# peterbudai/redux

Measured on NVIDIA B200. Metric: encode+decode round-trip throughput of raw input (bit-exact), higher is better.
Workload: dtype u32

## Files before the change

### redux_b200/csrc/redux_capi.cu

```cuda
#include <cuda_runtime.h>

#include <algorithm>
#include <chrono>
#include <atomic>
#include <condition_variable>
#include <deque>
#include <mutex>
#include <cstdio>
#include <cstdlib>
#include <cstring>
#include <string>
#include <thread>
#include <vector>

#include "../../include/redux_b200.h"
#include "redux_batch_kernels.cuh"
#include "redux_common.cuh"
#include "redux_lane_codec.cuh"
#include "redux_lane_al.cuh"
#include "redux_generic_codec.cuh"
#include "redux_warp_codec.cuh"
#include "redux_split_encoder.cuh"
#include "redux_train.cuh"

// ... 142 lines not shown
        release();
        cudaError_t e = cudaHostAlloc((void **)&buf, piece_bytes * (size_t)slots, cudaHostAllocDefault);
        if (e != cudaSuccess) { buf = nullptr; return e; }
        piece = piece_bytes; n = slots;
        ev.assign((size_t)slots, nullptr); recorded.assign((size_t)slots, 0);
        for (auto &x : ev) if ((e = cudaEventCreateWithFlags(&x, cudaEventDisableTiming)) != cudaSuccess) return e;
        return cudaSuccess;
    }
    void release() {
        for (auto x : ev) if (x) cudaEventDestroy(x);
        ev.clear(); recorded.clear();
        if (buf) cudaFreeHost(buf);
        buf = nullptr; piece = 0; n = 0;
    }
    uint8_t *slot(int i) const { return buf + (size_t)i * piece; }
};

struct StagingConfig {
    int enable = 1;
    size_t min_bytes = (size_t)8 << 20;
    size_t piece_bytes = (size_t)8 << 20;
    int slots = 4;
    int threads = 0;
};

struct DeviceState {
    int device = 0;
    cudaStream_t stream = nullptr;
    cudaStream_t pipe[kPipeStreams] = {};
    cudaStream_t copy = nullptr;
    cudaStream_t h2d = nullptr;
    HostBuf pin_off, pin_status, pin_aux0, pin_aux1;
    DevBuf slots, sizes, flag;
    DevBuf st_in, st_off, st_bmod, st_out, st_ooff, st_status, st_aux0, st_aux1, st_roff;
    DevBuf split_hist, split_pairs;
    DevBuf gen_tabs, gen_init, gen_freq, gen_start, gen_magic;
    DevBuf train_rows, train_sample;
    uint8_t *text_lut = nullptr;
    DevBuf corpus; uint64_t corpus_len = 0;
    std::vector<MagicEntry> magics;
    bool smem_set = false;
    cudaEvent_t ws_busy = nullptr;
    bool ws_recorded = false;
    StageRing *ring_up = nullptr, *ring_down = nullptr;
};

}

struct TimedSpan { cudaEvent_t a, b; int kind; int device; };

struct ModelArgs { bool on = false; const uint32_t *freqs = nullptr; uint32_t n = 0; const uint32_t *block_model = nullptr; };

struct redux_ctx {
    std::vector<DeviceState> devs;
    int sched = REDUX_SCHED_AUTO;
    std::string last_error;
    uint64_t launches = 0;
    bool timing = false;
    ModelArgs models;
    std::vector<TimedSpan> spans;
    StagingConfig staging;
    CopyPool *pool = nullptr;
    std::atomic<uint64_t> kernels_launched{0};
    void note_kernel(int id) { kernels_launched.fetch_or((uint64_t)1 << id, std::memory_order_relaxed); }
};

// ... 233 lines not shown
{
    job.magic = magic; job.f = pl.f; job.c = pl.c;
    job.tcap = pl.pretrained ? (uint32_t)(((uint64_t)1 << pl.f) - 1 - kNsym) : pl.tcap;
    job.one = pl.c <= 32 ? 1u << (32 - pl.c) : 0u;
    job.init_tree = nullptr; job.count0 = kNsym; job.eof_freq = 1;
    job.models = pl.models;
    job.models.block_model = pl.models.start ? block_model : nullptr;
    job.gf_m = pl.gf_m; job.gf_sh = pl.gf_sh;
}

KernelId pick_encoder(const Plan &pl)
{
    const bool c32 = pl.c == 32;
    if (pl.warp) return pl.cls == kNarrow ? kEncWarpNarrow : pl.cls == kWide ? kEncWarpWide : kEncWarpHuge;
    if (!pl.aligned) return pl.wide_table ? kEncHugeU32 : kEncHugeU16;
    if (pl.lane_cls == kNarrow) return kEncNarrow;
    if (pl.lane_cls == kWide) return c32 ? kEncWideU32C32 : kEncWideU32;
    if (pl.wide_table) return c32 ? kEncWideDU32C32 : kEncWideDU32;
    if (pl.full_table) return c32 ? kEncWideDU16FullC32 : kEncWideDU16Full;
    return c32 ? kEncWideDU16C32 : kEncWideDU16;
}
KernelId pick_decoder(const Plan &pl)
{
    const bool c32 = pl.c == 32;
    if (pl.warp) return pl.cls == kNarrow ? kDecWarpNarrow : pl.cls == kHuge ? kDecWarpHuge : c32 ? kDecWarpWideC32 : kDecWarpWide;
    if (!pl.aligned) return pl.wide_table ? kDecHugeU32 : kDecHugeU16;
    if (pl.lane_cls == kNarrow) return pl.c <= 16 ? kDecNarrowStg : kDecNarrow;
    if (pl.lane_cls == kWide) return c32 ? kDecWideU32C32 : kDecWideU32;
    if (pl.wide_table) return c32 ? kDecWideDU32C32 : kDecWideDU32;
    if (pl.full_table) return c32 ? kDecWideDU16FullC32 : kDecWideDU16Full;
    return c32 ? kDecWideDU16C32 : kDecWideDU16;
}

#define RDX_LAUNCH_LANE(id, name, kernel, TW) case id: kernel<<<lane_grid, kLaneThreads, lane_smem<TW>(), s>>>(job); return true;
#define RDX_LAUNCH_WARP(id, name, kernel) case id: kernel<<<warp_grid, kWarpCtaThreads, 0, s>>>(job); return true;
bool launch_coder(KernelId id, const LaneEncJob &job, cudaStream_t s)
{
    const uint32_t lane_grid = (uint32_t)((job.n_blocks + kLaneThreads - 1) / kLaneThreads);
    const uint32_t warp_grid = (uint32_t)((job.n_blocks + kWarpCtaWarps - 1) / kWarpCtaWarps);
    switch (id) {
    RDX_LANE_ENCODERS(RDX_LAUNCH_LANE)
    RDX_WARP_ENCODERS(RDX_LAUNCH_WARP)
    default: return false;
    }
}
bool launch_coder(KernelId id, const LaneDecJob &job, cudaStream_t s)
{
    const uint32_t lane_grid = (uint32_t)((job.n_blocks + kLaneThreads - 1) / kLaneThreads);
    const uint32_t warp_grid = (uint32_t)((job.n_blocks + kWarpCtaWarps - 1) / kWarpCtaWarps);
    switch (id) {
    RDX_LANE_DECODERS(RDX_LAUNCH_LANE)
    RDX_WARP_DECODERS(RDX_LAUNCH_WARP)
    default: return false;
    }
}
#undef RDX_LAUNCH_LANE
#undef RDX_LAUNCH_WARP

int launch_encode_split(redux_ctx *ctx, DeviceState *d, const Plan &pl, const LaneEncJob &job, cudaStream_t s, KernelId *kid)
{
    if (!d) return fail(ctx, REDUX_INVALID_INPUT, "device is not part of this context");
    SplitJob sj;
    sj.in = job.in; sj.in_off = job.in_off; sj.n_blocks = job.n_blocks;
    sj.chunks_per_stream = (uint32_t)((pl.max_len + kSplitChunk - 1) / kSplitChunk);
    sj.pair_stride = (pl.max_len + 31) & ~(uint64_t)31;
    sj.tcap = pl.tcap;
    const uint64_t chunks = job.n_blocks * sj.chunks_per_stream;
    CU_TRY(ctx, d->split_hist.reserve(chunks * 256 * sizeof(uint32_t)));
    CU_TRY(ctx, d->split_pairs.reserve(job.n_blocks * sj.pair_stride * sizeof(uint2)));
    sj.hist = (uint32_t *)d->split_hist.p; sj.pairs = (uint2 *)d->split_pairs.p;
    split_hist_kernel<<<(uint32_t)chunks, 256, 0, s>>>(sj);
    split_scan_kernel<<<(uint32_t)job.n_blocks, 256, 0, s>>>(sj);
    split_model_kernel<<<(uint32_t)((chunks + kSplitModelWarps - 1) / kSplitModelWarps), kSplitModelWarps * 32, 0, s>>>(sj);
    const uint32_t grid = (uint32_t)job.n_blocks;
    if (pl.cls == kNarrow)   { split_coder_kernel<kNarrow, false><<<grid, 32, 0, s>>>(job, sj); *kid = kSplitNarrow; }
    else if (pl.c == 32)     { split_coder_kernel<kWide, true><<<grid, 32, 0, s>>>(job, sj);    *kid = kSplitWideC32; }
    else                     { split_coder_kernel<kWide, false><<<grid, 32, 0, s>>>(job, sj);   *kid = kSplitWide; }
    ctx->launches += 3;
    return REDUX_OK;
}

int check_kind(redux_ctx *ctx, int kind)
{
    if (kind != REDUX_MODEL_LINEAR && kind != REDUX_MODEL_TREE)
        return fail(ctx, REDUX_INVALID_INPUT, "unknown model kind");
    return REDUX_OK;
}

struct DeviceGuard {
// ... 91 lines not shown

extern "C" uint32_t redux_debug_div_by_range(uint64_t x, uint64_t range) { return div_by_range64(x, range); }

extern "C" uint64_t redux_debug_magic_divide(uint64_t n, uint64_t magic, uint32_t shift, int wide)
{
    if (wide == 2) { Magic64 g{magic, shift, 0}; return div_magic65(n, g); }
    if (wide == 3) { union { double f; uint64_t u; } cv; cv.u = magic; MagicD g; g.r = cv.f; return div_magicd(n, g); }
    if (wide) { Magic64 g{magic, shift, 0}; return div_magic64(n, g); }
    Magic32 g{(uint32_t)magic, shift};
    return div_magic32((uint32_t)n, g);
}

extern "C" void redux_debug_renorm(uint64_t low, uint64_t high, uint32_t c, uint32_t *n1, uint32_t *k,
                                   uint64_t *nl, uint64_t *nh)
{
    if (c <= 32) { Renorm<uint32_t> r = renorm<uint32_t>((uint32_t)low, (uint32_t)high, c); *n1 = r.n1; *k = r.k; *nl = r.low; *nh = r.high; }
    else         { Renorm<uint64_t> r = renorm<uint64_t>(low, high, c); *n1 = r.n1; *k = r.k; *nl = r.low; *nh = r.high; }
}

extern "C" void redux_debug_shard(uint64_t n_blocks, uint32_t n_devices, uint32_t g, uint64_t *first, uint64_t *count)
{
    const uint64_t a = n_blocks * g / n_devices, b = n_blocks * (g + 1) / n_devices;
    *first = a; *count = b - a;
}

extern "C" int redux_debug_lane_occupancy(int *enc_ctas_per_sm, int *dec_ctas_per_sm)
{
    if (!enc_ctas_per_sm || !dec_ctas_per_sm) return REDUX_INVALID_INPUT;
    if (configure_kernels() != cudaSuccess) { (void)cudaGetLastError(); return REDUX_CUDA_ERROR; }
    const size_t s16 = (size_t)kLaneWarpsPerCta * kTabNodes * 32 * 2 + kTabPadBytes;
    if (cudaOccupancyMaxActiveBlocksPerMultiprocessor(enc_ctas_per_sm, encode_lane_al_kernel<uint16_t, kNarrow, true, false>,
                                                      kLaneThreads, s16) != cudaSuccess ||
        cudaOccupancyMaxActiveBlocksPerMultiprocessor(dec_ctas_per_sm, decode_lane_al_kernel<uint16_t, kNarrow, true, false, true>,
                                                      kLaneThreads, s16) != cudaSuccess) {
        (void)cudaGetLastError();
        return REDUX_CUDA_ERROR;
    }
    return REDUX_OK;
}

extern "C" const char *redux_debug_kernel_name(int id)
{
#define RDX_KERNEL_NAME(id, name, ...) name,
    static const char *const names[] = { RDX_ALL_KERNELS(RDX_KERNEL_NAME) };
#undef RDX_KERNEL_NAME
    return id >= 0 && id < kKernelIdCount ? names[id] : nullptr;
}

extern "C" int redux_debug_launched_kernels(redux_ctx_t *ctx, uint64_t *mask, int reset)
{
    if (!ctx || !mask) return REDUX_INVALID_INPUT;
    *mask = reset ? ctx->kernels_launched.exchange(0) : ctx->kernels_launched.load();
    return REDUX_OK;
}

extern "C" void redux_generate_blocks_host(uint8_t *out, uint64_t first_block, uint64_t n_blocks,
                                           uint64_t block_len, uint64_t seed)
{
    redux_generate_blocks_host_ex(out, first_block, n_blocks, block_len, seed, nullptr, 0);
}

extern "C" void redux_generate_blocks_host_ex(uint8_t *out, uint64_t first_block, uint64_t n_blocks,
                                              uint64_t block_len, uint64_t seed, const uint8_t *corpus, uint64_t corpus_len)
{
    uint8_t lut[256];
    for (uint32_t u = 0; u < 256; ++u) lut[u] = text_symbol(u);
    const uint64_t groups = (block_len + 7) >> 3;
// ... 62 lines not shown
                          cudaStreamCreateWithFlags(&d.copy, cudaStreamNonBlocking) == cudaSuccess &&
                          cudaStreamCreateWithFlags(&d.h2d, cudaStreamNonBlocking) == cudaSuccess;
        for (int i = 0; i < kPipeStreams && streams_ok; ++i)
            streams_ok = cudaStreamCreateWithFlags(&d.pipe[i], cudaStreamNonBlocking) == cudaSuccess;
        if (!streams_ok || cudaStreamCreateWithFlags(&d.stream, cudaStreamNonBlocking) != cudaSuccess ||
            configure_kernels() != cudaSuccess ||
            cudaMalloc((void **)&d.text_lut, 256) != cudaSuccess ||
            cudaMemcpy(d.text_lut, lut, 256, cudaMemcpyHostToDevice) != cudaSuccess) {
            (void)cudaGetLastError();
            ctx->devs.push_back(d);
            redux_ctx_destroy(ctx);
            return REDUX_CUDA_ERROR;
        }
        ctx->devs.push_back(d);
    }
    *out = ctx;
    return REDUX_OK;
}

extern "C" void redux_ctx_destroy(redux_ctx_t *ctx)
{
    if (!ctx) return;
    for (auto &d : ctx->devs) {
        DeviceGuard g(d.device);
        cudaDeviceSynchronize();
        if (d.ws_busy) cudaEventDestroy(d.ws_busy);
        if (d.stream) cudaStreamDestroy(d.stream);
        if (d.copy) cudaStreamDestroy(d.copy);
        if (d.h2d) cudaStreamDestroy(d.h2d);
        for (int i = 0; i < kPipeStreams; ++i) if (d.pipe[i]) cudaStreamDestroy(d.pipe[i]);
        for (HostBuf *b : {&d.pin_off, &d.pin_status, &d.pin_aux0, &d.pin_aux1}) b->release();
        for (DevBuf *b : {&d.slots, &d.sizes, &d.flag, &d.st_in, &d.st_off, &d.st_bmod, &d.st_out, &d.st_ooff,
                          &d.st_status, &d.st_aux0, &d.st_aux1, &d.st_roff, &d.corpus, &d.gen_magic, &d.gen_tabs, &d.gen_init,
                          &d.gen_freq, &d.gen_start, &d.split_hist, &d.split_pairs, &d.train_rows, &d.train_sample}) b->release();
        for (auto &m : d.magics) cudaFree(m.ptr);
        if (d.text_lut) cudaFree(d.text_lut);
        for (StageRing *r : {d.ring_up, d.ring_down}) if (r) { r->release(); delete r; }
    }
    delete ctx->pool;
    delete ctx;
}

extern "C" int redux_ctx_device_count(const redux_ctx_t *ctx) { return ctx ? (int)ctx->devs.size() : 0; }
extern "C" const char *redux_ctx_last_error(const redux_ctx_t *ctx) { return ctx ? ctx->last_error.c_str() : ""; }
extern "C" uint64_t redux_ctx_kernel_launches(const redux_ctx_t *ctx) { return ctx ? ctx->launches : 0; }

extern "C" int redux_ctx_timing_enable(redux_ctx_t *ctx, int on)
{
    if (!ctx) return REDUX_INVALID_INPUT;
    ctx->timing = on != 0;
    return REDUX_OK;
}

extern "C" int redux_ctx_timing_collect(redux_ctx_t *ctx, double *ms, uint64_t *counts)
{
    if (!ctx || !ms || !counts) return REDUX_INVALID_INPUT;
    for (int k = 0; k < REDUX_KERNEL_KINDS; ++k) { ms[k] = 0; counts[k] = 0; }
    int rc = REDUX_OK;
    for (auto &sp : ctx->spans) {
        DeviceGuard g(sp.device);
        float t = 0;
        if (cudaEventSynchronize(sp.b) == cudaSuccess && cudaEventElapsedTime(&t, sp.a, sp.b) == cudaSuccess) {
            ms[sp.kind] += t; counts[sp.kind] += 1;
        } else { (void)cudaGetLastError(); rc = REDUX_CUDA_ERROR; }
        cudaEventDestroy(sp.a); cudaEventDestroy(sp.b);
    }
    ctx->spans.clear();
// ... 73 lines not shown
        else if (pl.split) {
            DeviceState *d = find_dev(ctx, device);
            int rc = launch_encode_split(ctx, d, pl, job, s, &kid);
            if (rc) return rc;
        }
        else {
            kid = pick_encoder(pl);
            if (!launch_coder(kid, job, s)) return fail(ctx, REDUX_CUDA_ERROR, "no encoder for the plan");
        }
        ctx->note_kernel(kid);
    }
    ctx->launches++;
    CU_TRY(ctx, cudaGetLastError());
    {
        KernelTimer kt(ctx, device, s, REDUX_KERNEL_SCAN);
        scan_sizes_kernel<<<1, kScanThreads, 0, s>>>(sizes, n_blocks, d_out_off, out_capacity, flag);
    }
    ctx->launches++;
    CU_TRY(ctx, cudaGetLastError());
    const uint32_t cgrid = (uint32_t)std::min<uint64_t>(n_blocks, 148 * 16);
    {
        KernelTimer kt(ctx, device, s, REDUX_KERNEL_COMPACT);
        compact_kernel<<<cgrid, kCompactThreads, 0, s>>>(slots, pl.slot_stride, sizes, d_out_off, n_blocks,
                                                         d_out, out_capacity, d_status);
    }
    ctx->launches++;
    CU_TRY(ctx, cudaGetLastError());
    return REDUX_OK;
}

int decode_launch(redux_ctx *ctx, int device, cudaStream_t s, const Plan &pl, const void *magic,
                  const uint8_t *d_comp, const uint64_t *d_comp_off, const uint32_t *d_block_model, uint64_t n_blocks,
                  uint8_t *d_raw, const uint64_t *d_raw_off, uint64_t *d_raw_lens, uint64_t *d_consumed,
                  int32_t *d_status)
{
    LaneDecJob job;
    job.comp = d_comp; job.comp_off = d_comp_off; job.n_blocks = n_blocks;
    job.raw = d_raw; job.raw_off = d_raw_off; job.raw_len = d_raw_lens; job.consumed = d_consumed;
    job.status = d_status;
    set_plan_fields(job, pl, magic, d_block_model);
    {
        KernelTimer kt(ctx, device, s, REDUX_KERNEL_DECODE);
        KernelId kid;
        if (pl.generic) {
            GenericJob g = generic_job(pl, d_block_model);
            g.in = d_comp; g.in_off = d_comp_off; g.n_blocks = n_blocks;
            g.raw = d_raw; g.raw_off = d_raw_off; g.raw_len = d_raw_lens; g.consumed = d_consumed; g.status = d_status;
            decode_generic_kernel<<<pl.gen_threads / kGenericThreads, kGenericThreads, generic_smem_bytes(pl.s), s>>>(g);
            kid = pl.s <= kGenericSmemSymbolBits ? kDecGenericSmem : kDecGenericGlobal;
        }
        else {
            kid = pick_decoder(pl);
            if (!launch_coder(kid, job, s)) return fail(ctx, REDUX_CUDA_ERROR, "no decoder for the plan");
        }
        ctx->note_kernel(kid);
    }
    ctx->launches++;
    CU_TRY(ctx, cudaGetLastError());
    return REDUX_OK;
}

}

extern "C" int redux_encode_batch_device(redux_ctx_t *ctx, int device, void *stream_, int model_kind,
                                         const redux_params_t *params, const uint8_t *d_in,
                                         const uint64_t *d_in_offsets, uint64_t n_blocks,
                                         uint64_t max_block_len, uint8_t *d_out, uint64_t out_capacity,
                                         uint64_t *d_out_offsets, int32_t *d_status)
{
// ... 21 lines not shown
    CU_TRY(ctx, d->sizes.reserve(n_blocks * sizeof(uint32_t)));
    CU_TRY(ctx, d->flag.reserve(sizeof(int32_t)));
    rc = encode_launch(ctx, device, s, pl, magic, d_in, d_in_offsets, ctx->models.block_model, n_blocks, d_out, out_capacity,
                       d_out_offsets, d_status, (uint8_t *)d->slots.p, (uint32_t *)d->sizes.p,
                       (int32_t *)d->flag.p);
    CU_TRY(ctx, ws_release(d, s));
    return rc;
}

extern "C" int redux_decode_batch_device(redux_ctx_t *ctx, int device, void *stream_, int model_kind,
                                         const redux_params_t *params, const uint8_t *d_comp,
                                         const uint64_t *d_comp_offsets, uint64_t n_blocks,
                                         uint64_t max_block_len, uint8_t *d_raw,
                                         const uint64_t *d_raw_offsets, uint64_t *d_raw_lens,
                                         uint64_t *d_consumed, int32_t *d_status)
{
    if (!ctx) return REDUX_INVALID_INPUT;
    int rc;
    if ((rc = check_kind(ctx, model_kind))) return rc;
    Plan pl;
    if ((rc = make_plan(ctx, params, max_block_len, &pl))) return rc;
    pl.warp = !pl.generic && !pl.pretrained && choose_warp(ctx);
    DeviceState *d = find_dev(ctx, device);
    if (!d) return fail(ctx, REDUX_INVALID_INPUT, "device is not part of this context");
    if (n_blocks == 0) return REDUX_OK;
    if (!d_comp_offsets || !d_raw_offsets || !d_raw_lens || !d_consumed || !d_status)
        return fail(ctx, REDUX_INVALID_INPUT, "NULL buffer");
    DeviceGuard g(device);
    cudaStream_t s = (cudaStream_t)stream_;
    CU_TRY(ctx, ws_acquire(d, s));
    const void *magic = nullptr;
    if ((rc = get_magic(ctx, d, s, pl, &magic))) return rc;
    if ((rc = prepare_models(ctx, d, s, params, n_blocks, &pl))) return rc;
    rc = decode_launch(ctx, device, s, pl, magic, d_comp, d_comp_offsets, ctx->models.block_model, n_blocks, d_raw, d_raw_offsets,
                       d_raw_lens, d_consumed, d_status);
    CU_TRY(ctx, ws_release(d, s));
    return rc;
}

extern "C" int redux_generate_blocks_device(redux_ctx_t *ctx, int device, void *stream_, uint8_t *d_out,
                                            uint64_t first_block, uint64_t n_blocks, uint64_t block_len,
                                            uint64_t seed)
{
    if (!ctx) return REDUX_INVALID_INPUT;
    DeviceState *d = find_dev(ctx, device);
    if (!d) return fail(ctx, REDUX_INVALID_INPUT, "device is not part of this context");
    if (n_blocks == 0 || block_len == 0) return REDUX_OK;
    DeviceGuard g(device);
    cudaStream_t s = (cudaStream_t)stream_;
    {
        KernelTimer kt(ctx, device, s, REDUX_KERNEL_GENERATE);
        generate_kernel<<<148 * 8, 256, 0, s>>>(d_out, first_block, n_blocks, block_len, seed, d->text_lut,
                                                (const uint8_t *)d->corpus.p, d->corpus_len);
    }
    ctx->launches++;
    CU_TRY(ctx, cudaGetLastError());
    return REDUX_OK;
}

namespace {

struct Shard { uint64_t first, count; };

struct Trace {
    bool on; std::chrono::steady_clock::time_point t0;
    Trace() : on(std::getenv("REDUX_TRACE") != nullptr), t0(std::chrono::steady_clock::now()) {}
    void mark(const char *what, long k = -1) const {
        if (!on) return;
// ... 440 lines not shown
namespace {

int decode_shard(redux_ctx *ctx, DeviceState *d, const redux_params_t *p, const uint8_t *comp,
                 const uint64_t *comp_off, Shard sh, uint8_t *raw, const uint64_t *raw_off,
                 uint64_t *raw_lens, uint64_t *consumed, int32_t *status)
{
    Trace tr;
    DeviceGuard g(d->device);
    const uint64_t cbase = comp_off[sh.first], cbytes = comp_off[sh.first + sh.count] - cbase;
    const uint64_t rbase = raw_off[sh.first], rbytes = raw_off[sh.first + sh.count] - rbase;
    std::vector<uint64_t> rel(2 * (sh.count + 1));
    uint64_t *crel = rel.data(), *rrel = rel.data() + sh.count + 1;
    uint64_t max_len = 0;
    for (uint64_t i = 0; i <= sh.count; ++i) {
        crel[i] = comp_off[sh.first + i] - cbase;
        rrel[i] = raw_off[sh.first + i] - rbase;
        if (i) {
            if (crel[i] < crel[i - 1] || rrel[i] < rrel[i - 1]) return fail(ctx, REDUX_INVALID_INPUT, "offsets not monotonic");
            max_len = std::max(max_len, rrel[i] - rrel[i - 1]);
        }
    }
    Plan pl;
    int rc = make_plan(ctx, p, max_len, &pl);
    if (rc) return rc;
    pl.warp = !pl.generic && !pl.pretrained && choose_warp(ctx);
    const std::vector<Shard> chunks = pl.generic ? std::vector<Shard>{{0, sh.count}} : make_chunks(sh.count, -1);
    const size_t nc = chunks.size();
    CU_TRY(ctx, d->st_in.reserve(cbytes + 32));
    CU_TRY(ctx, d->st_off.reserve(rel.size() * sizeof(uint64_t)));
    CU_TRY(ctx, d->st_out.reserve(rbytes + 32));
    CU_TRY(ctx, d->st_aux0.reserve(sh.count * sizeof(uint64_t)));
    CU_TRY(ctx, d->st_aux1.reserve(sh.count * sizeof(uint64_t)));
    CU_TRY(ctx, d->st_status.reserve(sh.count * sizeof(int32_t)));
    CU_TRY(ctx, d->pin_aux0.reserve(sh.count * sizeof(uint64_t)));
    CU_TRY(ctx, d->pin_aux1.reserve(sh.count * sizeof(uint64_t)));
    CU_TRY(ctx, d->pin_status.reserve(sh.count * sizeof(int32_t)));
    const void *magic = nullptr;
    if ((rc = get_magic(ctx, d, d->pipe[0], pl, &magic))) return rc;
    if ((rc = prepare_models(ctx, d, d->pipe[0], p, sh.count, &pl))) return rc;
    EventSet evs;
    CU_TRY(ctx, evs.create(2 * nc));
    const bool stage_in = needs_staging(ctx, comp, cbytes), stage_out = needs_staging(ctx, raw, rbytes);
    const bool staged = stage_in || stage_out;
    if (stage_in) CU_TRY(ctx, ensure_ring(ctx, &d->ring_up));
    if (stage_out) CU_TRY(ctx, ensure_ring(ctx, &d->ring_down));
    CU_TRY(ctx, cudaMemcpyAsync(d->st_off.p, rel.data(), rel.size() * sizeof(uint64_t), cudaMemcpyHostToDevice, d->h2d));
    const uint32_t *d_bmod = nullptr;
    if ((rc = upload_block_models(ctx, d, sh, &d_bmod))) return rc;
    uint8_t *d_comp = (uint8_t *)d->st_in.p, *d_raw = (uint8_t *)d->st_out.p;
    uint64_t *d_coff = (uint64_t *)d->st_off.p, *d_roff = d_coff + sh.count + 1;
    uint64_t *d_len = (uint64_t *)d->st_aux0.p, *d_cons = (uint64_t *)d->st_aux1.p;
    int32_t *d_status = (int32_t *)d->st_status.p;
    uint64_t *h_len = (uint64_t *)d->pin_aux0.p, *h_cons = (uint64_t *)d->pin_aux1.p;
    int32_t *h_status = (int32_t *)d->pin_status.p;
    ChunkProgress prog;
    auto enqueue_all = [&]() -> int {
        int up_slot = 0;
        for (size_t k = 0; k < nc && !prog.stop.load(std::memory_order_relaxed); ++k) {
            const Shard c = chunks[k];
            cudaStream_t s = d->pipe[k % pipe_streams()];
            int rc2 = REDUX_OK;
            cudaError_t e = cudaSuccess;
            const uint64_t c0 = crel[c.first], c1 = crel[c.first + c.count];
            const uint64_t r0 = rrel[c.first], r1 = rrel[c.first + c.count];
            if (c1 > c0) e = stage_in ? staged_h2d(d->ring_up, ctx->pool, d->h2d, d_comp + c0, comp + cbase + c0, c1 - c0, &up_slot, &prog.stop)
                                      : cudaMemcpyAsync(d_comp + c0, comp + cbase + c0, c1 - c0, cudaMemcpyHostToDevice, d->h2d);
            if (e == cudaSuccess) e = cudaEventRecord(evs.ev[k], d->h2d);
            if (e == cudaSuccess) e = cudaStreamWaitEvent(s, evs.ev[k], 0);
            if (e == cudaSuccess)
                rc2 = decode_launch(ctx, d->device, s, pl, magic, d_comp, d_coff + c.first, d_bmod ? d_bmod + c.first : nullptr, c.count, d_raw,
                                    d_roff + c.first, d_len + c.first, d_cons + c.first, d_status + c.first);
            if (e == cudaSuccess && rc2 == REDUX_OK && stage_out) e = cudaEventRecord(evs.ev[nc + k], s);
            if (e == cudaSuccess && rc2 == REDUX_OK && !stage_out && r1 > r0)
                e = cudaMemcpyAsync(raw + rbase + r0, d_raw + r0, r1 - r0, cudaMemcpyDeviceToHost, s);
            if (e == cudaSuccess && rc2 == REDUX_OK)
                e = cudaMemcpyAsync(h_len + c.first, d_len + c.first, c.count * sizeof(uint64_t), cudaMemcpyDeviceToHost, s);
            if (e == cudaSuccess && rc2 == REDUX_OK)
                e = cudaMemcpyAsync(h_cons + c.first, d_cons + c.first, c.count * sizeof(uint64_t), cudaMemcpyDeviceToHost, s);
            if (e == cudaSuccess && rc2 == REDUX_OK)
                e = cudaMemcpyAsync(h_status + c.first, d_status + c.first, c.count * sizeof(int32_t), cudaMemcpyDeviceToHost, s);
            if (rc2 != REDUX_OK) return rc2;
            if (e != cudaSuccess) { (void)cudaGetLastError(); return fail(ctx, REDUX_CUDA_ERROR, "decode pipeline enqueue", e); }
            prog.advance();
        }
        return REDUX_OK;
    };
    int feeder_rc = REDUX_OK;
    std::thread feeder;
    if (staged) {
        feeder = std::thread([&] { DeviceGuard fg(d->device); feeder_rc = enqueue_all(); prog.finish(); });
    } else {
        feeder_rc = enqueue_all();
        prog.finish();
    }
    cudaError_t derr = cudaSuccess;
    if (stage_out) {
        DownStager down{d->ring_down, ctx->pool, d->copy, {}, 0};
        for (size_t k = 0; k < nc && derr == cudaSuccess; ++k) {
            if (!prog.wait_for(k)) break;
            const Shard c = chunks[k];
            const uint64_t r0 = rrel[c.first], r1 = rrel[c.first + c.count];
            if ((derr = cudaStreamWaitEvent(d->copy, evs.ev[nc + k], 0)) != cudaSuccess) break;
            if (r1 > r0) derr = down.push(raw + rbase + r0, d_raw + r0, r1 - r0);
        }
// ... 329 lines not shown
```

### redux_b200/csrc/redux_lane_al.cuh

```cuda
#pragma once
#include "redux_common.cuh"
#include "redux_lane_codec.cuh"

namespace rdx {

__device__ __forceinline__ uint32_t pinned(uint32_t x, uint64_t loaded_offset) { return x + (uint32_t)(loaded_offset >> 63); }
__device__ __forceinline__ uint64_t pinned(uint64_t x, uint64_t loaded_offset) { return x + (loaded_offset >> 63); }

__device__ __forceinline__ uint32_t clz_nz(uint32_t x) {
#if defined(__CUDA_ARCH__)
    uint32_t r;
    asm("bfind.shiftamt.u32 %0, %1;" : "=r"(r) : "r"(x));
    return r;
#else
    return (uint32_t)__builtin_clz(x);
#endif
}

__device__ __forceinline__ uint32_t clz_sh(uint32_t x) {
#if defined(__CUDA_ARCH__)
    return clz_nz(x);
#else
    return x ? (uint32_t)__builtin_clz(x) : 0xFFFFFFFFu;
#endif
// ... 215 lines not shown
    }
    __device__ __forceinline__ uint32_t finish() {
        const uint32_t bytes = wi * 4 + (nb + 7) / 8;
        if (nb) w0[wi] = __byte_perm((uint32_t)(acc << (32 - nb)), 0, 0x0123);
        return bytes;
    }
};

struct StageSlot {
#if defined(__CUDA_ARCH__)
    uint32_t sa;
    __device__ __forceinline__ void init(void *slot) { sa = (uint32_t)__cvta_generic_to_shared(slot); }
    __device__ __forceinline__ void request(const uint32_t *g) const {
        asm volatile("cp.async.ca.shared.global [%0], [%1], 4;" :: "r"(sa), "l"(g));
    }
    __device__ __forceinline__ uint32_t read() const {
        uint32_t v;
        asm volatile("ld.shared.u32 %0, [%1];" : "=r"(v) : "r"(sa));
        return v;
    }
    static __device__ __forceinline__ void commit() { asm volatile("cp.async.commit_group;"); }
    template <int KEEP> static __device__ __forceinline__ void wait() { asm volatile("cp.async.wait_group %0;" :: "n"(KEEP)); }
#else
    uint32_t val;
    void init(void *) { val = 0; }
    void request(const uint32_t *g) { val = *g; }
    uint32_t read() const { return val; }
    static void commit() {}
    template <int KEEP> static void wait() {}
#endif
};

template <typename TW>
__device__ __forceinline__ void *lane_stage_slot(void *smem) {
    return reinterpret_cast<uint8_t *>(smem) + (size_t)kLaneWarpsPerCta * kTabNodes * 32 * sizeof(TW) + kTabZeroRowBytes + threadIdx.x * 4;
}

struct ByteSource3 {
    const uint32_t *base;
    uint32_t wi, wlast;
    uint32_t cur;
    uint32_t pos;
    StageSlot slot;

    __device__ __forceinline__ void request() {
        slot.request(base + (wi < wlast ? wi : wlast));
        ++wi;
    }
    __device__ __forceinline__ void init(const uint8_t *src, uint32_t len, void *slot_mem) {
        const uintptr_t a = (uintptr_t)src;
        base = reinterpret_cast<const uint32_t *>(a & ~(uintptr_t)3);
        pos = (uint32_t)(a & 3);
        wlast = len ? (pos + len - 1) >> 2 : 0;
        wi = 1;
        cur = 0;
        slot.init(slot_mem);
        if (len) {
            cur = __ldg(base) >> (8 * pos);
            request();
            StageSlot::commit();
        }
    }
    __device__ __forceinline__ void refill() {
        StageSlot::wait<0>();
        cur = slot.read();
        request();
        StageSlot::commit();
    }
// ... 72 lines not shown
            magic += (int32_t)(count0 - job.count0);
            tcap = job.tcap + job.count0 - count0;
        }
        return ok;
    }
};

template <typename TW, int CLS, bool FULL, bool C32>
__global__ void __launch_bounds__(kLaneThreads, 2)
encode_lane_al_kernel(const LaneEncJob job)
{
    using C = Cls<CLS>;
    using M = typename C::M;
    extern __shared__ uint4 smem_u4[];
    const uint32_t lane = threadIdx.x & 31, warp = threadIdx.x >> 5;
    const uint64_t blk = (uint64_t)blockIdx.x * kLaneThreads + threadIdx.x;
    if (blk >= job.n_blocks) return;

    StreamStart<M> st;
    const bool valid = st.init(job, blk);
    LaneTable2<TW, FULL> tab;
    tab.init(smem_u4, warp, lane);
    tab.reset(st.tree);

    const uint64_t off = job.in_off[blk];
    const uint32_t len = valid ? (uint32_t)(job.in_off[blk + 1] - off) : 0u;
    const uint32_t c = job.c, sh = 32 - c;
    const uint32_t one = pinned(job.one, off);
    const uint32_t count0 = st.count0, eof_freq = st.eof_freq;
    const M *magic = st.magic;
    const uint32_t tcap = st.tcap;

    ByteSource3 src;
    src.init(job.in + off, len, lane_stage_slot<TW>(smem_u4));
    BitSink2 sink;
    sink.init(job.slots + blk * job.slot_stride);
    uint32_t L = 0, H = 0xFFFFFFFFu;
    uint32_t pend = 0;

    const uint32_t n_adapt = len < tcap ? len : tcap;
    uint32_t t = 0;
    M gn = C::ldm(magic);
    auto adapt_coded = [&](uint32_t sym, const M &g) {
        uint32_t cl, ch;
        tab.template query<true>(sym, count0 + t - eof_freq - (FULL ? 0u : 256u), cl, ch);
        encode_step_al<CLS, C32>(L, H, pend, sink, cl, ch, count0 + t, g, sh, one);
        ++t;
    };
    auto adapt_core = [&](uint32_t sym, const M &g) {
        uint32_t cl, ch;
        tab.template query<true>(sym, count0 + t - eof_freq - (FULL ? 0u : 256u), cl, ch);
        const BitSink2::Code cd = encode_core_al<CLS, C32>(L, H, cl, ch, count0 + t, g, sh, one);
        ++t;
        return cd;
    };
    auto adapt_step = [&](uint32_t sym) {
        const M g = gn;
        gn = C::ldm(magic + t + 1);
        adapt_coded(sym, g);
    };
    while (t < n_adapt && !src.word_aligned()) adapt_step(src.next());
    if (t + 4 <= n_adapt) {
        M g0 = gn, g1 = C::ldm(magic + t + 1), g2 = C::ldm(magic + t + 2), g3 = C::ldm(magic + t + 3);
        while (t + 4 <= n_adapt) {
            const M m0 = C::ldm(magic + t + 4), m1 = C::ldm(magic + t + 5), m2 = C::ldm(magic + t + 6), m3 = C::ldm(magic + t + 7);
            const uint32_t wv = src.take_word();
            const BitSink2::Code c0 = adapt_core(__byte_perm(wv, 0, 0x4440), g0), c1 = adapt_core(__byte_perm(wv, 0, 0x4441), g1);
// ... 43 lines not shown
    sink.put_code(top_bits(L, extra), extra, pend, 0);
    const uint32_t bytes = sink.finish();
    job.sizes[blk] = valid ? bytes : 0u;
    job.status[blk] = valid ? 0 : kStatusInvalidInput;
    StageSlot::wait<0>();
}

struct BitWindow {
    uint32_t w0, w1, w2, pos;
    const uint32_t *base;
    uint32_t idx, last;
    StageSlot slot;

    static __device__ __forceinline__ uint32_t swap(uint32_t x) { return __byte_perm(x, 0, 0x0123); }
    __device__ __forceinline__ uint32_t word_at(uint32_t i) const { return __ldg(base + (i < last ? i : last)); }
    __device__ __forceinline__ void request() {
        slot.request(base + (idx < last ? idx : last));
        ++idx;
    }
    __device__ __forceinline__ uint32_t init(const uint8_t *src, uint32_t len, void *slot_mem) {
        const uintptr_t a = (uintptr_t)src;
        const uint32_t mis = (uint32_t)(a & 3);
        base = reinterpret_cast<const uint32_t *>(a & ~(uintptr_t)3);
        last = ((mis + len + 3) >> 2) - 1;
        pos = 8 * mis;
        slot.init(slot_mem);
        w0 = swap(word_at(0)); w1 = swap(word_at(1));
        const uint32_t first = win();
        w0 = w1; w1 = swap(word_at(2)); w2 = swap(word_at(3));
        idx = 4;
        request();
        StageSlot::commit();
        return first;
    }
    __device__ __forceinline__ uint32_t win() const { return __funnelshift_l(w1, w0, pos); }
    __device__ __forceinline__ uint32_t win2() const {
        const bool up = pos >= 32;
        return __funnelshift_l(up ? w2 : w1, up ? w1 : w0, pos);
    }
    __device__ __forceinline__ void skip(uint32_t n) { pos += n; }
    __device__ __forceinline__ void advance(uint32_t n) {
        StageSlot::wait<0>();
        pos += n;
        if (pos >= 32) { pos -= 32; w0 = w1; w1 = w2; w2 = swap(slot.read()); request(); }
        StageSlot::commit();
    }
};

struct BitWindowReg {
    uint32_t w0, w1, nxt, pos;
    const uint32_t *base;
    uint32_t idx, last;

    static __device__ __forceinline__ uint32_t swap(uint32_t x) { return __byte_perm(x, 0, 0x0123); }
    __device__ __forceinline__ uint32_t ld() {
        const uint32_t v = __ldg(base + (idx < last ? idx : last));
        ++idx;
        return v;
    }
    __device__ __forceinline__ uint32_t init(const uint8_t *src, uint32_t len) {
        const uintptr_t a = (uintptr_t)src;
        const uint32_t mis = (uint32_t)(a & 3);
        base = reinterpret_cast<const uint32_t *>(a & ~(uintptr_t)3);
        last = ((mis + len + 3) >> 2) - 1;
        idx = 0;
        pos = 8 * mis;
// ... 261 lines not shown
            if (t < t_end) (void)step<ADAPT, true>(sym, ADAPT ? C::ldm(magic + t) : g_frozen, count_frozen);
            return;
        }
        M g0 = ADAPT ? C::ldm(magic + t) : g_frozen, g1 = g0, g2 = g0, g3 = g0;
        if (ADAPT) { g1 = C::ldm(magic + t + 1); g2 = C::ldm(magic + t + 2); g3 = C::ldm(magic + t + 3); }
        while (t + 4 <= t_end) {
            M m0 = g0, m1 = g1, m2 = g2, m3 = g3;
            if (ADAPT) {
                m0 = C::ldm(magic + t + 4); m1 = C::ldm(magic + t + 5); m2 = C::ldm(magic + t + 6); m3 = C::ldm(magic + t + 7);
            }
            constexpr int M1 = STG ? 1 : 0, M2 = STG ? 2 : 0;
            uint32_t wv;
            if (!step<ADAPT, false, M1>(sym, g0, count_frozen)) break;
            wv = sym;
            if (!step<ADAPT, false, M2>(sym, g1, count_frozen)) { out.partial(wv, 1); break; }
            wv |= sym << 8;
            if (!step<ADAPT, false, M1>(sym, g2, count_frozen)) { out.partial(wv, 2); break; }
            wv |= sym << 16;
            if (!step<ADAPT, false, M2>(sym, g3, count_frozen)) { out.partial(wv, 3); break; }
            out.put4(wv | (sym << 24));
            if (ADAPT) { g0 = m0; g1 = m1; g2 = m2; g3 = m3; }
        }
        M gn = g0;
        while (st == 0 && t < t_end) {
            const M g = gn;
            if (ADAPT) gn = C::ldm(magic + t + 1);
            if (!step<ADAPT, false>(sym, g, count_frozen)) break;
            out.put(sym);
        }
        if (ADAPT) { tab.t[128 << 5] = (TW)top_a; tab.t[64 << 5] = (TW)top_b; tab.t[192 << 5] = (TW)top_c; }
    }
};

template <typename TW, int CLS, bool FULL, bool C32, bool STG>
__global__ void __launch_bounds__(kLaneThreads, 2)
decode_lane_al_kernel(const LaneDecJob job)
{
    using D = LaneDecoderAl<TW, CLS, FULL, C32, STG>;
    using M = typename D::M;
    extern __shared__ uint4 smem_u4[];
    const uint32_t lane = threadIdx.x & 31, warp = threadIdx.x >> 5;
    const uint64_t blk = (uint64_t)blockIdx.x * kLaneThreads + threadIdx.x;
    D d;
    d.tab.init(smem_u4, warp, lane);
    if (D::kFrozenCum) {
        reinterpret_cast<uint32_t *>(d.tab.t)[0] = 0u;
        if (warp == kLaneWarpsPerCta - 1)
            reinterpret_cast<uint32_t *>(reinterpret_cast<uint8_t *>(smem_u4) + (size_t)kLaneWarpsPerCta * kTabNodes * 32 * sizeof(TW))[lane] = 0u;
        __syncthreads();
    }
    if (blk >= job.n_blocks) return;
    StreamStart<M> st;
    const bool valid = st.init(job, blk);
    d.tab.reset(st.tree);

    const uint64_t coff = job.comp_off[blk];
    const uint64_t clen = valid ? job.comp_off[blk + 1] - coff : 0u;
    const uint64_t roff = job.raw_off[blk];
    const uint64_t cap64 = valid ? job.raw_off[blk + 1] - roff : 0u;
    if (clen >= (1ull << 29)) {
        job.raw_len[blk] = 0; job.consumed[blk] = 0; job.status[blk] = 5;
        return;
    }
    const uint32_t c = job.c;
    const uint32_t cap = cap64 > 0xFFFFFFFEull ? 0xFFFFFFFEu : (uint32_t)cap64;
    const uint32_t total_bits = (uint32_t)clen * 8;
    d.sh = 32 - c; d.one = job.one; d.count0 = st.count0; d.eof_freq = st.eof_freq;
    uint32_t *scratch = reinterpret_cast<uint32_t *>(job.consumed + blk);
    d.out.init(job.raw + roff, scratch);
    d.st = 0; d.t = 0;
    d.L = 0; d.H = 0xFFFFFFFFu; d.V = 0; d.left = 0;
    const M *magic = st.magic;
    const uint32_t tcap = st.tcap;

    if (total_bits < c) {
        d.st = 1;
    } else {
        d.V = d.bw.init(job.comp + coff, (uint32_t)clen, lane_stage_slot<TW>(smem_u4));
        d.left = total_bits - c;
    }
    const M g0 = D::C::ldm(magic);
    const uint32_t e1 = d.st != 0 ? 0u : (tcap < cap ? tcap : cap);
    d.template run<true, false>(e1, magic, 0, g0);
    if (d.st == 0 && d.t == cap && cap < tcap) d.template run<true, true>(d.t + 1, magic, 0, g0);
    const M gf = D::C::mk(job.gf_m, job.gf_sh);
    if (D::kFrozenCum && d.st == 0) d.tab.freeze_to_cumulative();
    d.template run<false, false>(d.st != 0 ? d.t : cap, magic, d.count0 + tcap, gf);
    if (d.st == 0) d.template run<false, true>(d.t + 1, magic, d.count0 + tcap, gf);
    d.out.finish(scratch);
    job.raw_len[blk] = d.t;
    job.consumed[blk] = (total_bits - d.left + 7) >> 3;
    job.status[blk] = !valid ? kStatusInvalidInput : d.st < 0 ? 0 : d.st;
    StageSlot::wait<0>();
}

}
```

### redux_b200/csrc/redux_lane_codec.cuh

```cuda
#pragma once
#include "redux_common.cuh"

namespace rdx {

constexpr int kLaneWarpsPerCta = 7;
constexpr int kLaneThreads = kLaneWarpsPerCta * 32;
constexpr int kTabNodes = 256;
constexpr int kTabZeroRowBytes = 128;
constexpr int kTabPadBytes = kTabZeroRowBytes + kLaneThreads * 4;

struct BlockModels {
    const uint32_t *trees = nullptr;
    const uint2 *start = nullptr;
    const uint32_t *block_model = nullptr;
    uint32_t n_models = 0;
};
constexpr int32_t kStatusInvalidInput = 2;

__device__ __forceinline__ bool block_row(const BlockModels &bm, uint64_t blk, uint32_t &m) {
    m = bm.block_model ? __ldg(bm.block_model + blk) : 0u;
    return m < bm.n_models;
}

struct LaneEncJob {
    const uint8_t *in;
    const uint64_t *in_off;
    uint64_t n_blocks;
    uint8_t *slots;
    uint64_t slot_stride;
    uint32_t *sizes;
    int32_t *status;
    const void *magic;
    uint32_t f, c;
    uint32_t tcap;
    uint32_t one;
    const uint32_t *init_tree;
    uint32_t count0;
    uint32_t eof_freq;
    BlockModels models;
    uint64_t gf_m; uint32_t gf_sh;
};

struct LaneDecJob {
    const uint8_t *comp;
    const uint64_t *comp_off;
    uint64_t n_blocks;
    uint8_t *raw;
    const uint64_t *raw_off;
    uint64_t *raw_len;
    uint64_t *consumed;
    int32_t *status;
    const void *magic;
    uint32_t f, c;
    uint32_t tcap;
    uint32_t one;
    const uint32_t *init_tree;
    uint32_t count0, eof_freq;
    BlockModels models;
    uint64_t gf_m; uint32_t gf_sh;
};

template <int CLS> struct Cls;
template <> struct Cls<kNarrow> {
    using S = uint32_t; using P = uint32_t; using M = Magic32;
    static __device__ __forceinline__ P mulr(uint32_t v, S rm1) { return v * rm1 + v; }
    static __device__ __forceinline__ P mul_add(uint32_t v, S rm1, P acc) { return v * (rm1 + 1u) + acc; }
    static __device__ __forceinline__ P divc(P n, const M &g, uint32_t) { return div_magic32(n, g); }
    static __device__ __forceinline__ M ldm(const M *p) {
        uint2 v = __ldg(reinterpret_cast<const uint2 *>(p)); M g; g.m = v.x; g.sh = v.y; return g;
    }
    static __device__ __forceinline__ M mk(uint64_t m, uint32_t sh) { M g; g.m = (uint32_t)m; g.sh = sh; return g; }
};
template <> struct Cls<kWide> {
    using S = uint32_t; using P = uint64_t; using M = Magic64;
    static __device__ __forceinline__ P mulr(uint32_t v, S rm1) { return (uint64_t)v * rm1 + v; }
    static __device__ __forceinline__ P mul_add(uint32_t v, S rm1, P acc) { return (uint64_t)v * rm1 + (acc + v); }
    static __device__ __forceinline__ P divc(P n, const M &g, uint32_t) { return div_magic64(n, g); }
    static __device__ __forceinline__ M ldm(const M *p) {
        uint4 v = __ldg(reinterpret_cast<const uint4 *>(p));
        M g; g.m = ((uint64_t)v.y << 32) | v.x; g.sh = v.z; g.pad = 0; return g;
    }
    static __device__ __forceinline__ M mk(uint64_t m, uint32_t sh) { M g; g.m = m; g.sh = sh; g.pad = 0; return g; }
};
template <> struct Cls<kWideD> {
    using S = uint32_t; using P = uint64_t; using M = MagicD;
    static __device__ __forceinline__ P mulr(uint32_t v, S rm1) { return (uint64_t)v * rm1 + v; }
    static __device__ __forceinline__ P mul_add(uint32_t v, S rm1, P acc) { return (uint64_t)v * rm1 + (acc + v); }
    static __device__ __forceinline__ P divc(P n, const M &g, uint32_t) { return div_magicd(n, g); }
    static __device__ __forceinline__ M ldm(const M *p) { M g; g.r = __ldg(reinterpret_cast<const double *>(p)); return g; }
    static __device__ __forceinline__ M mk(uint64_t bits, uint32_t) {
        M g;
#if defined(__CUDA_ARCH__)
// ... 402 lines not shown
```

Before: 117,300.

## Split lane decoding into resumable chunks with a per-CTA warp work queue

The lane decoder becomes resumable. Each stream decodes a fixed number of symbols per chunk, then saves its coder, bit reader and output state to a global record. An extra worker warp per CTA (8 warps for 7 groups) pulls unfinished groups from a shared-memory queue and continues them, so an idle warp can pick up lagging streams and latency is hidden better. The cost is extra state save and restore traffic to global memory, atomics and spin waits on the queue, and the risk of divergent warps handing groups back and forth.

```diff
diff --git a/redux_b200/csrc/redux_capi.cu b/redux_b200/csrc/redux_capi.cu
--- a/redux_b200/csrc/redux_capi.cu
+++ b/redux_b200/csrc/redux_capi.cu
@@ -198,6 +198,7 @@
     cudaStream_t h2d = nullptr;
     HostBuf pin_off, pin_status, pin_aux0, pin_aux1;
     DevBuf slots, sizes, flag;
+    DevBuf dec_hand;
     DevBuf st_in, st_off, st_bmod, st_out, st_ooff, st_status, st_aux0, st_aux1, st_roff;
     DevBuf split_hist, split_pairs;
     DevBuf gen_tabs, gen_init, gen_freq, gen_start, gen_magic;
@@ -497,7 +498,10 @@
     return c32 ? kDecWideDU16C32 : kDecWideDU16;
 }
 
+constexpr uint32_t lane_decoder_threads(KernelId id) { return id == kDecHugeU16 || id == kDecHugeU32 ? kLaneThreads : kLaneWorkerThreads; }
+
 #define RDX_LAUNCH_LANE(id, name, kernel, TW) case id: kernel<<<lane_grid, kLaneThreads, lane_smem<TW>(), s>>>(job); return true;
+#define RDX_LAUNCH_LANE_DEC(id, name, kernel, TW) case id: kernel<<<lane_grid, lane_decoder_threads(id), lane_smem<TW>(), s>>>(job); return true;
 #define RDX_LAUNCH_WARP(id, name, kernel) case id: kernel<<<warp_grid, kWarpCtaThreads, 0, s>>>(job); return true;
 bool launch_coder(KernelId id, const LaneEncJob &job, cudaStream_t s)
 {
@@ -514,12 +518,13 @@
     const uint32_t lane_grid = (uint32_t)((job.n_blocks + kLaneThreads - 1) / kLaneThreads);
     const uint32_t warp_grid = (uint32_t)((job.n_blocks + kWarpCtaWarps - 1) / kWarpCtaWarps);
     switch (id) {
-    RDX_LANE_DECODERS(RDX_LAUNCH_LANE)
+    RDX_LANE_DECODERS(RDX_LAUNCH_LANE_DEC)
     RDX_WARP_DECODERS(RDX_LAUNCH_WARP)
     default: return false;
     }
 }
 #undef RDX_LAUNCH_LANE
+#undef RDX_LAUNCH_LANE_DEC
 #undef RDX_LAUNCH_WARP
 
 int launch_encode_split(redux_ctx *ctx, DeviceState *d, const Plan &pl, const LaneEncJob &job, cudaStream_t s, KernelId *kid)
@@ -677,7 +682,7 @@
     if (cudaOccupancyMaxActiveBlocksPerMultiprocessor(enc_ctas_per_sm, encode_lane_al_kernel<uint16_t, kNarrow, true, false>,
                                                       kLaneThreads, s16) != cudaSuccess ||
         cudaOccupancyMaxActiveBlocksPerMultiprocessor(dec_ctas_per_sm, decode_lane_al_kernel<uint16_t, kNarrow, true, false, true>,
-                                                      kLaneThreads, s16) != cudaSuccess) {
+                                                      kLaneWorkerThreads, s16) != cudaSuccess) {
         (void)cudaGetLastError();
         return REDUX_CUDA_ERROR;
     }
@@ -806,7 +811,7 @@
         for (HostBuf *b : {&d.pin_off, &d.pin_status, &d.pin_aux0, &d.pin_aux1}) b->release();
         for (DevBuf *b : {&d.slots, &d.sizes, &d.flag, &d.st_in, &d.st_off, &d.st_bmod, &d.st_out, &d.st_ooff,
                           &d.st_status, &d.st_aux0, &d.st_aux1, &d.st_roff, &d.corpus, &d.gen_magic, &d.gen_tabs, &d.gen_init,
-                          &d.gen_freq, &d.gen_start, &d.split_hist, &d.split_pairs, &d.train_rows, &d.train_sample}) b->release();
+                          &d.gen_freq, &d.gen_start, &d.split_hist, &d.split_pairs, &d.train_rows, &d.train_sample, &d.dec_hand}) b->release();
         for (auto &m : d.magics) cudaFree(m.ptr);
         if (d.text_lut) cudaFree(d.text_lut);
         for (StageRing *r : {d.ring_up, d.ring_down}) if (r) { r->release(); delete r; }
@@ -946,9 +951,10 @@
 int decode_launch(redux_ctx *ctx, int device, cudaStream_t s, const Plan &pl, const void *magic,
                   const uint8_t *d_comp, const uint64_t *d_comp_off, const uint32_t *d_block_model, uint64_t n_blocks,
                   uint8_t *d_raw, const uint64_t *d_raw_off, uint64_t *d_raw_lens, uint64_t *d_consumed,
-                  int32_t *d_status)
+                  int32_t *d_status, LaneDecRec *d_hand)
 {
     LaneDecJob job;
+    job.hand = d_hand;
     job.comp = d_comp; job.comp_off = d_comp_off; job.n_blocks = n_blocks;
     job.raw = d_raw; job.raw_off = d_raw_off; job.raw_len = d_raw_lens; job.consumed = d_consumed;
     job.status = d_status;
@@ -1036,8 +1042,9 @@
     const void *magic = nullptr;
     if ((rc = get_magic(ctx, d, s, pl, &magic))) return rc;
     if ((rc = prepare_models(ctx, d, s, params, n_blocks, &pl))) return rc;
+    CU_TRY(ctx, d->dec_hand.reserve(n_blocks * sizeof(LaneDecRec)));
     rc = decode_launch(ctx, device, s, pl, magic, d_comp, d_comp_offsets, ctx->models.block_model, n_blocks, d_raw, d_raw_offsets,
-                       d_raw_lens, d_consumed, d_status);
+                       d_raw_lens, d_consumed, d_status, (LaneDecRec *)d->dec_hand.p);
     CU_TRY(ctx, ws_release(d, s));
     return rc;
 }
@@ -1544,6 +1551,7 @@
     CU_TRY(ctx, d->st_aux0.reserve(sh.count * sizeof(uint64_t)));
     CU_TRY(ctx, d->st_aux1.reserve(sh.count * sizeof(uint64_t)));
     CU_TRY(ctx, d->st_status.reserve(sh.count * sizeof(int32_t)));
+    CU_TRY(ctx, d->dec_hand.reserve(sh.count * sizeof(LaneDecRec)));
     CU_TRY(ctx, d->pin_aux0.reserve(sh.count * sizeof(uint64_t)));
     CU_TRY(ctx, d->pin_aux1.reserve(sh.count * sizeof(uint64_t)));
     CU_TRY(ctx, d->pin_status.reserve(sh.count * sizeof(int32_t)));
@@ -1581,7 +1589,8 @@
             if (e == cudaSuccess) e = cudaStreamWaitEvent(s, evs.ev[k], 0);
             if (e == cudaSuccess)
                 rc2 = decode_launch(ctx, d->device, s, pl, magic, d_comp, d_coff + c.first, d_bmod ? d_bmod + c.first : nullptr, c.count, d_raw,
-                                    d_roff + c.first, d_len + c.first, d_cons + c.first, d_status + c.first);
+                                    d_roff + c.first, d_len + c.first, d_cons + c.first, d_status + c.first,
+                                    (LaneDecRec *)d->dec_hand.p + c.first);
             if (e == cudaSuccess && rc2 == REDUX_OK && stage_out) e = cudaEventRecord(evs.ev[nc + k], s);
             if (e == cudaSuccess && rc2 == REDUX_OK && !stage_out && r1 > r0)
                 e = cudaMemcpyAsync(raw + rbase + r0, d_raw + r0, r1 - r0, cudaMemcpyDeviceToHost, s);
diff --git a/redux_b200/csrc/redux_lane_al.cuh b/redux_b200/csrc/redux_lane_al.cuh
--- a/redux_b200/csrc/redux_lane_al.cuh
+++ b/redux_b200/csrc/redux_lane_al.cuh
@@ -271,8 +271,8 @@
 };
 
 template <typename TW>
-__device__ __forceinline__ void *lane_stage_slot(void *smem) {
-    return reinterpret_cast<uint8_t *>(smem) + (size_t)kLaneWarpsPerCta * kTabNodes * 32 * sizeof(TW) + kTabZeroRowBytes + threadIdx.x * 4;
+__device__ __forceinline__ void *lane_stage_slot(void *smem, uint32_t stream) {
+    return reinterpret_cast<uint8_t *>(smem) + (size_t)kLaneWarpsPerCta * kTabNodes * 32 * sizeof(TW) + kTabZeroRowBytes + stream * 4;
 }
 
 struct ByteSource3 {
@@ -411,7 +411,7 @@
     const uint32_t tcap = st.tcap;
 
     ByteSource3 src;
-    src.init(job.in + off, len, lane_stage_slot<TW>(smem_u4));
+    src.init(job.in + off, len, lane_stage_slot<TW>(smem_u4, threadIdx.x));
     BitSink2 sink;
     sink.init(job.slots + blk * job.slot_stride);
     uint32_t L = 0, H = 0xFFFFFFFFu;
@@ -521,6 +521,14 @@
         request();
         StageSlot::commit();
         return first;
+    }
+    __device__ __forceinline__ void resume(const uint8_t *src, uint32_t len, void *slot_mem) {
+        const uintptr_t a = (uintptr_t)src;
+        base = reinterpret_cast<const uint32_t *>(a & ~(uintptr_t)3);
+        last = ((uint32_t)(a & 3) + len + 3) / 4 - 1;
+        slot.init(slot_mem);
+        slot.request(base + (idx - 1 < last ? idx - 1 : last));
+        StageSlot::commit();
     }
     __device__ __forceinline__ uint32_t win() const { return __funnelshift_l(w1, w0, pos); }
     __device__ __forceinline__ uint32_t win2() const {
@@ -848,66 +856,180 @@
     }
 };
 
+enum : uint32_t { kDecStart = 0, kDecAdapt = 1, kDecFrozen = 2, kDecDone = 3 };
+
 template <typename TW, int CLS, bool FULL, bool C32, bool STG>
-__global__ void __launch_bounds__(kLaneThreads, 2)
-decode_lane_al_kernel(const LaneDecJob job)
+__device__ __forceinline__ bool decode_lane_chunk(const LaneDecJob &job, void *smem, uint32_t stream, uint64_t blk,
+                                                  LaneDecRec &rec, uint32_t t_stop)
 {
     using D = LaneDecoderAl<TW, CLS, FULL, C32, STG>;
     using M = typename D::M;
-    extern __shared__ uint4 smem_u4[];
-    const uint32_t lane = threadIdx.x & 31, warp = threadIdx.x >> 5;
-    const uint64_t blk = (uint64_t)blockIdx.x * kLaneThreads + threadIdx.x;
+    if (rec.phase == kDecDone) return true;
     D d;
-    d.tab.init(smem_u4, warp, lane);
-    if (D::kFrozenCum) {
-        reinterpret_cast<uint32_t *>(d.tab.t)[0] = 0u;
-        if (warp == kLaneWarpsPerCta - 1)
-            reinterpret_cast<uint32_t *>(reinterpret_cast<uint8_t *>(smem_u4) + (size_t)kLaneWarpsPerCta * kTabNodes * 32 * sizeof(TW))[lane] = 0u;
-        __syncthreads();
-    }
-    if (blk >= job.n_blocks) return;
+    d.tab.init(smem, stream >> 5, stream & 31);
     StreamStart<M> st;
     const bool valid = st.init(job, blk);
-    d.tab.reset(st.tree);
-
     const uint64_t coff = job.comp_off[blk];
     const uint64_t clen = valid ? job.comp_off[blk + 1] - coff : 0u;
     const uint64_t roff = job.raw_off[blk];
     const uint64_t cap64 = valid ? job.raw_off[blk + 1] - roff : 0u;
-    if (clen >= (1ull << 29)) {
-        job.raw_len[blk] = 0; job.consumed[blk] = 0; job.status[blk] = 5;
-        return;
-    }
     const uint32_t c = job.c;
     const uint32_t cap = cap64 > 0xFFFFFFFEull ? 0xFFFFFFFEu : (uint32_t)cap64;
     const uint32_t total_bits = (uint32_t)clen * 8;
     d.sh = 32 - c; d.one = job.one; d.count0 = st.count0; d.eof_freq = st.eof_freq;
     uint32_t *scratch = reinterpret_cast<uint32_t *>(job.consumed + blk);
     d.out.init(job.raw + roff, scratch);
-    d.st = 0; d.t = 0;
-    d.L = 0; d.H = 0xFFFFFFFFu; d.V = 0; d.left = 0;
+    void *slot = lane_stage_slot<TW>(smem, stream);
     const M *magic = st.magic;
     const uint32_t tcap = st.tcap;
-
-    if (total_bits < c) {
-        d.st = 1;
+    uint32_t phase = rec.phase;
+    if (phase == kDecStart) {
+        d.tab.reset(st.tree);
+        if (clen >= (1ull << 29)) {
+            job.raw_len[blk] = 0; job.consumed[blk] = 0; job.status[blk] = 5;
+            rec.phase = kDecDone;
+            return true;
+        }
+        d.st = 0; d.t = 0;
+        d.L = 0; d.H = 0xFFFFFFFFu; d.V = 0; d.left = 0;
+        if (total_bits < c) {
+            d.st = 1;
+        } else {
+            d.V = d.bw.init(job.comp + coff, (uint32_t)clen, slot);
+            d.left = total_bits - c;
+        }
+        phase = kDecAdapt;
     } else {
-        d.V = d.bw.init(job.comp + coff, (uint32_t)clen, lane_stage_slot<TW>(smem_u4));
-        d.left = total_bits - c;
+        d.st = 0; d.t = rec.t;
+        d.L = rec.L; d.H = rec.H; d.V = rec.V; d.left = rec.left;
+        d.bw.w0 = rec.w0; d.bw.w1 = rec.w1; d.bw.w2 = rec.w2; d.bw.pos = rec.pos; d.bw.idx = rec.idx;
+        d.bw.resume(job.comp + coff, (uint32_t)clen, slot);
+        d.out.top = rec.top; d.out.c8 = rec.c8;
+        d.out.pw = d.out.w0 + rec.pw;
+        d.out.wp = (rec.pw == 0 && d.out.ph) ? scratch : d.out.pw;
     }
     const M g0 = D::C::ldm(magic);
-    const uint32_t e1 = d.st != 0 ? 0u : (tcap < cap ? tcap : cap);
-    d.template run<true, false>(e1, magic, 0, g0);
-    if (d.st == 0 && d.t == cap && cap < tcap) d.template run<true, true>(d.t + 1, magic, 0, g0);
     const M gf = D::C::mk(job.gf_m, job.gf_sh);
-    if (D::kFrozenCum && d.st == 0) d.tab.freeze_to_cumulative();
-    d.template run<false, false>(d.st != 0 ? d.t : cap, magic, d.count0 + tcap, gf);
-    if (d.st == 0) d.template run<false, true>(d.t + 1, magic, d.count0 + tcap, gf);
+    bool more = false;
+    if (phase == kDecAdapt) {
+        const uint32_t e1 = d.st != 0 ? 0u : (tcap < cap ? tcap : cap);
+        d.template run<true, false>(e1 < t_stop ? e1 : t_stop, magic, 0, g0);
+        more = d.st == 0 && d.t < e1;
+        if (!more) {
+            if (d.st == 0 && d.t == cap && cap < tcap) d.template run<true, true>(d.t + 1, magic, 0, g0);
+            if (D::kFrozenCum && d.st == 0) d.tab.freeze_to_cumulative();
+            phase = kDecFrozen;
+        }
+    }
+    if (phase == kDecFrozen) {
+        const uint32_t e2 = d.st != 0 ? d.t : cap;
+        d.template run<false, false>(e2 < t_stop ? e2 : t_stop, magic, d.count0 + tcap, gf);
+        more = d.st == 0 && d.t < e2;
+        if (!more && d.st == 0) d.template run<false, true>(d.t + 1, magic, d.count0 + tcap, gf);
+    }
+    StageSlot::wait<0>();
+    if (more) {
+        rec.phase = phase; rec.t = d.t;
+        rec.L = d.L; rec.H = d.H; rec.V = d.V; rec.left = d.left;
+        rec.w0 = d.bw.w0; rec.w1 = d.bw.w1; rec.w2 = d.bw.w2; rec.pos = d.bw.pos; rec.idx = d.bw.idx;
+        rec.top = d.out.top; rec.c8 = d.out.c8; rec.pw = (uint32_t)(d.out.pw - d.out.w0);
+        return false;
+    }
     d.out.finish(scratch);
     job.raw_len[blk] = d.t;
     job.consumed[blk] = (total_bits - d.left + 7) >> 3;
     job.status[blk] = !valid ? kStatusInvalidInput : d.st < 0 ? 0 : d.st;
-    StageSlot::wait<0>();
-}
-
-}
+    rec.phase = kDecDone;
+    return true;
+}
+
+#if defined(__CUDA_ARCH__)
+struct GroupQueue {
+    static constexpr uint32_t kExit = 7;
+    uint32_t *w;
+    __device__ __forceinline__ static uint32_t entry(uint32_t p, uint32_t tok) { return (0x8000u | (p & 0xFFFu) << 3 | tok) << 16; }
+    __device__ __forceinline__ void init() { for (int i = 0; i < 32; ++i) w[i] = 0; }
+    __device__ __forceinline__ uint32_t take() {
+        const uint32_t p = atomicAdd(&w[0], 1u << 16) >> 16;
+        volatile uint32_t *e = &w[16 + (p & 15)];
+        uint32_t ns = 32;
+        for (;;) {
+            const uint32_t v = *e;
+            if (v == entry(p, (v >> 16) & 7u)) { *e = 0; __threadfence(); return (v >> 16) & 7u; }
+            __nanosleep(ns);
+            ns = ns < 1024 ? 2 * ns : ns;
+        }
+    }
+    __device__ __forceinline__ void push(uint32_t tok) {
+        const uint32_t p = atomicAdd(&w[1], 1u << 16) >> 16;
+        volatile uint32_t *e = &w[16 + (p & 15)];
+        while (*e != 0) __nanosleep(64);
+        __threadfence();
+        *e = entry(p, tok);
+    }
+    __device__ __forceinline__ uint32_t finished() { return atomicAdd(&w[2], 1u << 16) >> 16; }
+};
+#endif
+
+template <typename TW, int CLS, bool FULL, bool C32, bool STG>
+__global__ void __launch_bounds__(kLaneWorkerThreads, 2)
+decode_lane_al_kernel(const LaneDecJob job)
+{
+    using D = LaneDecoderAl<TW, CLS, FULL, C32, STG>;
+    extern __shared__ uint4 smem_u4[];
+    uint32_t *zero_row = reinterpret_cast<uint32_t *>(reinterpret_cast<uint8_t *>(smem_u4) + (size_t)kLaneWarpsPerCta * kTabNodes * 32 * sizeof(TW));
+    const uint32_t lane = threadIdx.x & 31;
+    const uint64_t blk0 = (uint64_t)blockIdx.x * kLaneThreads;
+    if (D::kFrozenCum) {
+        for (uint32_t i = threadIdx.x; i < (uint32_t)kLaneThreads; i += blockDim.x)
+            reinterpret_cast<uint32_t *>(smem_u4)[(size_t)(i >> 5) * kTabNodes * 32 * sizeof(TW) / 4 + (i & 31)] = 0u;
+        if (blockDim.x == (uint32_t)kLaneThreads && threadIdx.x < 32) zero_row[lane] = 0u;
+    }
+#if defined(__CUDA_ARCH__)
+    if (blockDim.x != (uint32_t)kLaneThreads) {
+        GroupQueue q{zero_row};
+        if (threadIdx.x == 0) q.init();
+        __syncthreads();
+        uint32_t g = threadIdx.x >> 5;
+        bool first = g < (uint32_t)kLaneWarpsPerCta;
+        for (;;) {
+            if (!first) {
+                g = lane == 0 ? q.take() : 0u;
+                g = __shfl_sync(0xFFFFFFFFu, g, 0);
+                if (g == GroupQueue::kExit) return;
+                __threadfence();
+            }
+            const uint32_t stream = g * 32 + lane;
+            const uint64_t blk = blk0 + stream;
+            bool done = blk >= job.n_blocks;
+            if (!done) {
+                LaneDecRec &rec = job.hand[blk];
+                if (first) rec.phase = kDecStart;
+                done = decode_lane_chunk<TW, CLS, FULL, C32, STG>(job, smem_u4, stream, blk, rec, first ? kLaneChunk : rec.t + kLaneChunk);
+            }
+            first = false;
+            const bool all = __all_sync(0xFFFFFFFFu, done);
+            __threadfence();
+            __syncwarp();
+            if (lane == 0) {
+                if (!all) q.push(g);
+                else if (q.finished() == (uint32_t)kLaneWarpsPerCta - 1)
+                    for (uint32_t i = kLaneWarpsPerCta; i < blockDim.x / 32; ++i) q.push(GroupQueue::kExit);
+            }
+            if (all) return;
+        }
+    }
+#endif
+    __syncthreads();
+    const uint32_t stream = threadIdx.x;
+    const uint64_t blk = blk0 + stream;
+    if (blk >= job.n_blocks) return;
+    LaneDecRec local;
+    LaneDecRec &rec = job.hand ? job.hand[blk] : local;
+    rec.phase = kDecStart;
+    uint32_t t_stop = 0;
+    do t_stop += kLaneChunk;
+    while (!decode_lane_chunk<TW, CLS, FULL, C32, STG>(job, smem_u4, stream, blk, rec, t_stop));
+}
+
+}
diff --git a/redux_b200/csrc/redux_lane_codec.cuh b/redux_b200/csrc/redux_lane_codec.cuh
--- a/redux_b200/csrc/redux_lane_codec.cuh
+++ b/redux_b200/csrc/redux_lane_codec.cuh
@@ -8,6 +8,13 @@
 constexpr int kTabNodes = 256;
 constexpr int kTabZeroRowBytes = 128;
 constexpr int kTabPadBytes = kTabZeroRowBytes + kLaneThreads * 4;
+constexpr int kLaneWorkers = 8;
+constexpr int kLaneWorkerThreads = kLaneWorkers * 32;
+#ifndef RDX_LANE_CHUNK
+#define RDX_LANE_CHUNK 2048
+#endif
+constexpr uint32_t kLaneChunk = RDX_LANE_CHUNK;
+static_assert(kLaneChunk % 4 == 0, "chunks end on the decoder's 4-symbol rounds");
 
 struct BlockModels {
     const uint32_t *trees = nullptr;
@@ -41,6 +48,13 @@
     uint64_t gf_m; uint32_t gf_sh;
 };
 
+struct alignas(16) LaneDecRec {
+    uint32_t L, H, V, t, left, phase;
+    uint32_t w0, w1, w2, pos, idx;
+    uint32_t top, c8, pw;
+    uint32_t pad[2];
+};
+
 struct LaneDecJob {
     const uint8_t *comp;
     const uint64_t *comp_off;
@@ -58,6 +72,7 @@
     uint32_t count0, eof_freq;
     BlockModels models;
     uint64_t gf_m; uint32_t gf_sh;
+    LaneDecRec *hand = nullptr;
 };
 
 template <int CLS> struct Cls;
```

Result: faster. 120,100, median of 6 (+2.5%).
